# cgbur/llama2.zig

Measured on AMD Instinct MI355X. Metric: tokens/s (argmax, -t 0), higher is better.
Workload: dtype f32; 1 GPU; llama2-7b shape, fp32 llama2.c-v0 checkpoint (dim 4096, hidden 11008, L 32, H 32, kv 32, V 32000, S 2048), greedy from BOS, seeded synthetic weights; parallelism=1 GPU

## Files before the change

### llama2.zig_amd/csrc/kernel_common.h

```cpp
#pragma once
#include <cstdlib>

#include "l2z_comm.h"
#include "l2z_internal.h"
#include "tunables.h"

namespace l2z {
namespace {

constexpr int kWave = 64;
constexpr int kBlock = 256;
constexpr int kWaves = kBlock / kWave;
constexpr int kScratch = 32;

typedef float v4f __attribute__((ext_vector_type(4)));
typedef float v2f __attribute__((ext_vector_type(2)));

__device__ __forceinline__ v4f ldg_nt(const v4f *p) { return __builtin_nontemporal_load(p); }

__device__ __forceinline__ void block_copy_row(float *dst, const float *src, const int n, const int tid, const int n_threads)
{
    const int n4 = ((((uintptr_t)src | (uintptr_t)dst) & 15) == 0) ? n >> 2 : 0;
    for (int i = tid; i < n4; i += n_threads) ((v4f *)dst)[i] = ((const v4f *)src)[i];
    for (int i = 4 * n4 + tid; i < n; i += n_threads) dst[i] = src[i];
// ... 135 lines not shown
            ss = fmaf(v.x, v.x, ss);
            ss = fmaf(v.y, v.y, ss);
            ss = fmaf(v.z, v.z, ss);
            ss = fmaf(v.w, v.w, ss);
        }
    }
    if (PRO == PRO_RMS) {
        ss = wave_sum(ss);
        if ((tid & 63) == 0) scratch[tid >> 6] = ss;
        __syncthreads();
        float tot = scratch[0];
#pragma unroll
        for (int i = 1; i < kWaves; i++) tot += scratch[i];
        float s = tot / (float)n;
        s += 1e-5f;
        s = 1.0f / sqrtf(s);
        const v4f *g4 = (const v4f *)rms_w;
#pragma unroll
        for (int k = 0; k < XC; k++) {
            const int j = tid + kBlock * k;
            if (j < n4) {
                v4f v = xr[k];
                v.x = (v.x * s) * gr[k].x;
                v.y = (v.y * s) * gr[k].y;
                v.z = (v.z * s) * gr[k].z;
                v.w = (v.w * s) * gr[k].w;
                xs4[j] = v;
            }
        }
        for (int j = tid + kBlock * XC; j < n4; j += kBlock) {
            v4f v = xs4[j];
            const v4f g = g4[j];
            v.x = (v.x * s) * g.x;
            v.y = (v.y * s) * g.y;
            v.z = (v.z * s) * g.z;
            v.w = (v.w * s) * g.w;
            xs4[j] = v;
        }
    }
    __syncthreads();
}

template <int PRO, int XC>
__device__ __forceinline__ void xstage_finish(const float *__restrict__ x,
                                              const float *__restrict__ rms_w, int n, int n4_pad,
                                              v4f (&xr)[XC], v4f (&gr)[XC], float *xs,
                                              float *scratch)
{
    const v4f *x4 = (const v4f *)x;
    xstage_tail<PRO, XC>(rms_w, n, n4_pad, xr, gr, xs, scratch, [&](int j) { return x4[j]; });
}

struct LLPoll {
    const unsigned long long *slot;
    unsigned e;
    unsigned count;
    int *ctl;
    int *h_err;
    long long timeout_ticks;
};

__device__ __forceinline__ LLPoll ll_poll_init(const LLIn &in)
{
    LLPoll p;
    const int e = in.ctl[kCtlEpoch] + in.gi;
    p.e = (unsigned)e;
    p.slot = in.slots + (size_t)(e & 1) * in.slot_floats;
    p.count = in.count;
    p.ctl = in.ctl;
    p.h_err = in.h_err;
    p.timeout_ticks = in.timeout_ticks;
    return p;
}

__device__ __forceinline__ v4f ll_wait4(const LLPoll &p, int j, v4u a, v4u b)
{
    if (!(ll_ready2(a, p.e) && ll_ready2(b, p.e))) {
        bool give_up = __hip_atomic_load(p.ctl + kCtlErr, __ATOMIC_RELAXED, __HIP_MEMORY_SCOPE_AGENT) != 0;
        const long long t0 = wall_clock64();
        while (!give_up) {
            __builtin_amdgcn_s_sleep(16);
            a = ll_load2(p.slot, (size_t)4 * j);
            b = ll_load2(p.slot, (size_t)4 * j + 2);
            if (ll_ready2(a, p.e) && ll_ready2(b, p.e)) break;
            if (wall_clock64() - t0 > p.timeout_ticks) {
                give_up = true;
                __hip_atomic_store(p.ctl + kCtlErr, 1, __ATOMIC_RELAXED, __HIP_MEMORY_SCOPE_AGENT);
                *p.h_err = 1 + (int)((unsigned)(4 * j) / (p.count ? p.count : 1u));
            }
        }
    }
    v4f v;
    v.x = __uint_as_float(a.x);
    v.y = __uint_as_float(a.z);
    v.z = __uint_as_float(b.x);
    v.w = __uint_as_float(b.z);
    return v;
}

template <int PRO, int XC>
__device__ __forceinline__ void xload_issue_ll(const LLPoll &p, const float *__restrict__ rms_w,
                                               int n4, v4u (&xl)[2 * XC], v4f (&gr)[XC])
{
    const v4f *g4 = (const v4f *)rms_w;
#pragma unroll
    for (int k = 0; k < XC; k++) {
        const int j = threadIdx.x + kBlock * k;
        const int jc = j < n4 ? j : 0;
        xl[2 * k] = ll_load2(p.slot, (size_t)4 * jc);
        xl[2 * k + 1] = ll_load2(p.slot, (size_t)4 * jc + 2);
    }
    if (PRO == PRO_RMS) {
#pragma unroll
        for (int k = 0; k < XC; k++) {
            const int j = threadIdx.x + kBlock * k;
            gr[k] = (j < n4) ? g4[j] : v4f{0.f, 0.f, 0.f, 0.f};
        }
    }
}

template <int PRO, int XC>
__device__ __forceinline__ void xstage_finish_ll(const LLPoll &p, const float *__restrict__ rms_w,
                                                 int n, int n4_pad, v4u (&xl)[2 * XC],
                                                 v4f (&gr)[XC], float *xs, float *scratch)
{
    const int n4 = n >> 2;
    v4f xr[XC];
#pragma unroll
    for (int k = 0; k < XC; k++) {
        const int j = threadIdx.x + kBlock * k;
        const v4f v = ll_wait4(p, j < n4 ? j : 0, xl[2 * k], xl[2 * k + 1]);
        xr[k] = (j < n4) ? v : v4f{0.f, 0.f, 0.f, 0.f};
    }
    xstage_tail<PRO, XC>(rms_w, n, n4_pad, xr, gr, xs, scratch, [&](int j) {
        return ll_wait4(p, j, ll_load2(p.slot, (size_t)4 * j), ll_load2(p.slot, (size_t)4 * j + 2));
    });
}

template <int PRO, int XC, bool LL>
struct XStage {
    v4f xr[LL ? 1 : XC], gr[XC];
    v4u xl[LL ? 2 * XC : 2];
    LLPoll poll;

    __device__ __forceinline__ void issue(const float *x, const LLIn &xin, const float *rms_w, int n4)
    {
        if constexpr (LL) {
            poll = ll_poll_init(xin);
            xload_issue_ll<PRO, XC>(poll, rms_w, n4, xl, gr);
        } else {
            xload_issue<PRO, XC>(x, rms_w, n4, xr, gr);
        }
    }
    __device__ __forceinline__ void finish(const float *x, const float *rms_w, int n, int n4_pad, float *xs, float *scratch)
    {
        if constexpr (LL)
            xstage_finish_ll<PRO, XC>(poll, rms_w, n, n4_pad, xl, gr, xs, scratch);
        else
            xstage_finish<PRO, XC>(x, rms_w, n, n4_pad, xr, gr, xs, scratch);
    }
};

__device__ __forceinline__ void block_softmax(float *att, int T, float *scratch)
{
    const int tid = threadIdx.x, nt = blockDim.x;
    float m = -INFINITY;
    for (int t = tid; t < T; t += nt) m = fmaxf(m, att[t]);
    m = block_max(m, scratch);
    float s = 0.0f;
    for (int t = tid; t < T; t += nt) {
        const float e = expf(att[t] - m);
        att[t] = e;
        s += e;
    }
    s = block_sum(s, scratch);
    for (int t = tid; t < T; t += nt) att[t] = att[t] / s;
    __syncthreads();
}

struct AttnGeom {
    int E;
    int TPR;
    int G;
};

__host__ __device__ inline AttnGeom attn_geom(int head_size, bool vec, int block = kBlock)
{
    AttnGeom g;
    g.E = vec ? head_size >> 2 : head_size;
    int t = 1;
    while (t < g.E && t < 64) t <<= 1;
    g.TPR = t;
    g.G = block / t;
    return g;
}

__device__ __forceinline__ void wave_softmax(const float *att, float *prob, int T)
{
    const int lane = threadIdx.x & 63, wave = threadIdx.x >> 6, nw = blockDim.x >> 6;
    float m = -INFINITY;
    for (int t = lane; t < T; t += kWave) m = fmaxf(m, att[t]);
    m = wave_max(m);
    float s = 0.0f;
    for (int t = lane; t < T; t += kWave) s += expf(att[t] - m);
    s = wave_sum(s);
    for (int t = wave * kWave + lane; t < T; t += nw * kWave) prob[t] = expf(att[t] - m) / s;
    __syncthreads();
}

inline bool aligned16(const void *p) { return (reinterpret_cast<uintptr_t>(p) & 15u) == 0; }

template <typename K>
hipError_t ensure_lds(K kernel, size_t bytes)
{
    if (bytes > 64 * 1024) {
        hipError_t e = hipFuncSetAttribute(reinterpret_cast<const void *>(kernel),
                                           hipFuncAttributeMaxDynamicSharedMemorySize, (int)bytes);
        if (e != hipSuccess) return e;
    }
    return hipSuccess;
}

template <typename K, typename... Args>
hipError_t launch_lds(K kernel, dim3 grid, dim3 block, size_t lds, hipStream_t st, Args... args)
{
    hipError_t e = ensure_lds(kernel, lds);
    if (e != hipSuccess) return e;
    hipLaunchKernelGGL(kernel, grid, block, lds, st, args...);
    return hipGetLastError();
}

}
}
```

### llama2.zig_amd/csrc/l2z_internal.h

```cpp
#pragma once

#include <hip/hip_runtime.h>

#include <cstdarg>
#include <cstdint>
#include <cstdio>
#include <string>
#include <vector>

#include "../../include/llama2_hip.h"
#include "../../include/llama2_hip_test.h"

namespace l2z {

struct P2pArgs;

struct LLIn {
    const unsigned long long *slots;
    unsigned slot_floats;
    unsigned count;
    int gi;
    int *ctl;
    int *h_err;
    long long timeout_ticks;
};

void set_error(const char *fmt, ...);

#define L2Z_HIP(expr)                                                                    \
    do {                                                                                 \
        hipError_t _e = (expr);                                                          \
        if (_e != hipSuccess) {                                                          \
            ::l2z::set_error("%s failed: %s (%s:%d)", #expr, hipGetErrorString(_e),      \
                             __FILE__, __LINE__);                                        \
            return _e == hipErrorOutOfMemory ? L2Z_ERR_OOM                               \
                   : (_e == hipErrorNoDevice || _e == hipErrorInvalidDevice)             \
                       ? L2Z_ERR_NO_DEVICE                                               \
                       : L2Z_ERR_HIP;                                                    \
        }                                                                                \
    } while (0)

#define L2Z_CHECK(cond, code, ...)          \
    do {                                    \
        if (!(cond)) {                      \
            ::l2z::set_error(__VA_ARGS__);  \
            return (code);                  \
        }                                   \
    } while (0)

#define L2Z_TRY(expr)              \
    do {                           \
        int _s = (expr);           \
        if (_s != L2Z_OK) return _s; \
    } while (0)

template <class Sig> class FnRef;
template <class R, class... Args> class FnRef<R(Args...)> {
  public:
    template <class F>
    FnRef(const F &f) : f_(&f), call_([](const void *p, Args... args) -> R { return (*(const F *)p)(args...); }) {}
    R operator()(Args... args) const { return call_(f_, args...); }

  private:
    const void *f_;
    R (*call_)(const void *, Args...);
};


enum Prologue { PRO_NONE = 0, PRO_RMS = 1 };
enum Epilogue { EPI_STORE = 0, EPI_ROPE = 1, EPI_RESID = 2, EPI_SWIGLU = 3, EPI_ARGMAX = 4 };

constexpr int kMaxSeg = 3;

struct ArgmaxArgs {
    const float *logits;
    int vocab;
    const float *part_val;
    const int *part_idx;
    int n_part;
    int *token_ptr;
    int *pos_ptr;
    const int *prompt;
    const int *n_prompt_ptr;
    int *out_tokens;
    int *argmax_out;
    const float *tok_emb;
    float *x;
    int dim;
    int advance;
    int *epoch_ctl;
    int epoch_add;
    const P2pArgs *xchg;
    int xchg_gi;
};

struct MatvecArgs {
    const float *w0, *w1, *w2;
    float *out0, *out1, *out2;
    int rows0, rows1, rows2;
    int pos_stride1, pos_stride2;
    size_t kv_head_stride;
    int n;
    const float *x;
    const float *rms_w;
    const float *resid;
    const int *pos_ptr;
    const float2 *rope;
    int head_size;
    int rope_segs;
    float *part_val;
    int *part_idx;
    int row_offset;
    const P2pArgs *push;
    const int *push_ctl;
    int push_gi;
    LLIn xin;
    const uint32_t *pk, *pk1, *pk2;
    int pk_e, pk_e1, pk_e2;
    int tl_slot;
};

struct AttnArgs {
    const float *q;
    const float *kcache;
    const float *vcache;
    float *xb;
    const int *pos_ptr;
    int head_size;
    int kv_row;
    size_t kv_head;
    int kv_mul;
    int seq_len;
    const P2pArgs *push;
    const int *push_ctl;
    int push_gi;
    int tl_seq;
};


struct FusedQkvAttnArgs {
    const float *wq, *wk, *wv;
    const float *rms_w, *x;
    float *q_out;
    float *kcache, *vcache;
    float *xb;
    const int *pos_ptr;
    const float2 *rope;
    int n;
    int head_size, seq_len, kv_dim;
    int kv_row;
    size_t kv_head;
};
bool fused_qkv_attn_supported(int dim, int n_heads, int n_kv_heads, int seq_len, int n_cus);
hipError_t launch_fused_qkv_attn(const FusedQkvAttnArgs &a, int n_heads, hipStream_t st);

hipError_t launch_pk_stats(const float *m, size_t count, uint32_t *stats, hipStream_t st);
hipError_t launch_pk_pack(const float *m, int rows, int n, int e_base, uint32_t *pk, hipStream_t st);
hipError_t launch_pk_unpack(const uint32_t *pk, int rows, int n, int e_base, float *out, hipStream_t st);
hipError_t launch_matvec(const MatvecArgs &a, int pro, int epi, int max_blocks_per_cu, int n_cus,
                         hipStream_t st, int *out_grid = nullptr, bool *pushed = nullptr);
bool attention_push_supported(const AttnArgs &a);
int matvec_max_grid(int n_cus);
bool matvec_vector_width(int n);
hipError_t launch_stream_read(const float *p, size_t n_floats, float *out, int n_cus, hipStream_t st);
hipError_t launch_attention(const AttnArgs &a, int n_heads_local, hipStream_t st, int form = 0);
int attention_short_pos(int head_size, int seq_len);
int attention_split_chunks(int n_heads_local, int n_cus);
size_t attention_split_part_floats(int n_heads_local, int head_size, int nch);
bool attention_split_supported(const AttnArgs &a);
hipError_t launch_attention_split(const AttnArgs &a, int n_heads_local, int nch, float *part,
                                  int *arrivals, hipStream_t st, bool small = false);
int attention_split_wide_pos(int seq_len);
hipError_t launch_argmax(const ArgmaxArgs &a, hipStream_t st);
hipError_t launch_set_state(int token, int pos, int *token_ptr, int *pos_ptr, const float *tok_emb,
                            float *x, int dim, hipStream_t st);
hipError_t launch_rmsnorm(float *o, const float *x, const float *w, int n, hipStream_t st);
hipError_t launch_softmax(float *x, int n, hipStream_t st);
hipError_t launch_probs(float *probs, const float *logits, int n, float temperature, hipStream_t st);
hipError_t launch_dot(float *out, const float *x, const float *y, int n, hipStream_t st);
hipError_t launch_weighted_sum_rows(float *xout, int xout_len, const float *rows, int row_stride,
                                    const float *weights, int n_weights, hipStream_t st);
hipError_t launch_synth_fill(float *dst, uint64_t base_idx, uint64_t count, uint64_t seed,
                             float scale, float bias, hipStream_t st, uint64_t row_len = 0, uint64_t row_pitch = 0,
                             uint64_t idx_pitch = 0);
hipError_t launch_sum_parts(float *out, const float *const *parts, int n_parts, int n, hipStream_t st);
hipError_t launch_copy_rows(float *dst, size_t dpitch, const float *src, size_t rows, size_t cols, hipStream_t st);
size_t attention_lds_bytes(int head_size, int seq_len, bool vec);

struct SplitKWs {
    float *part;
    int *cnt;
    size_t part_floats;
    int cnt_ints;
    void *x3;
    size_t x3_bytes;
    void *x3b;
    size_t x3b_bytes;
};
struct DeferredSum {
    const float *part;
    int sk, feat, tm;
    bool valid;
};
enum PlanesReady { PLANES_SPLIT = 0, PLANES_READY = 1, PLANES_READY_B = 2 };
constexpr int kSplitKMaxTokens = 256;
constexpr int kPanelWsRows = 6 * kSplitKMaxTokens;
int prefill_split_k(long long n_whole, int P, int K, bool pair);
enum PrefillGemmEpi { PG_STORE = 0, PG_RESID = 1, PG_ROPE = 2, PG_ROPE_CACHE = 3, PG_CACHE = 4,
                      PG_SWIGLU = 5 };
bool x3_applies(long long n_whole, int K);
bool x3_stream_shape(long long n_whole, int P, int K);
int x3_stream_sk(long long n_whole, int P, int K);
enum GemmKind { GEMM_SINGLE = 0,
                GEMM_QKV,
                GEMM_W13,
                GEMM_KV };
struct GemmShape {
    int kind, epi;
    int P, N, K, ldx;
    int n_scale;
    long long n_launch_whole;
    int sk;
    int nq, nkv;
    int w13_one_matrix;
    size_t part_floats;
    int cnt_ints;
};
enum GemmFamily { GF_INVALID = -1, GF_NOT_SUPPORTED = -2, GF_NO_WORKSPACE = -3,
                  GF_STREAM = 1,
                  GF_SHORT,
                  GF_SPLIT_K,
                  GF_TWO_BLOCK,
                  GF_TILE };
enum TileForm { TILE_128x64 = 0, TILE_64x64, TILE_32x64, TILE_32x32, TILE_128x128 };
struct GemmPlan {
    int family;
    int epi;
    int K;
    int x3;
    int sk;
    int tile;
    int feat, tm, nbuf, one_round;
    int tms, paired;
};
GemmPlan prefill_gemm_plan(const GemmShape &s);
hipError_t launch_prefill_rmsnorm(float *o, int ldo, const float *x, const float *w, int n, int P,
                                  hipStream_t st,
                                  void *x3 = nullptr, int kp = 0,
                                  const DeferredSum *pending = nullptr,
                                  const int *rows = nullptr);
hipError_t launch_prefill_embed(float *x, const float *tok_emb, const int *tokens, int dim, int P,
                                hipStream_t st);
hipError_t launch_prefill_attention(const float *q, int ldq, const float *kcache, const float *vcache,
                                    float *out, int ldo, int pos0, int P, int n_heads, int head_size,
                                    int kv_row, size_t kv_head, int kv_mul, int seq_len, hipStream_t st,
                                    int n_heads_model = 0,
                                    int form = 0,
                                    void *x3 = nullptr, int kp = 0,
                                    bool *planes_written = nullptr);
constexpr int kRaggedMaxSeq = 16;
struct RaggedSeq {
    float *kc, *vc;
    int row0, rows;
    int pos0;
    int pad;
    const int32_t *pages;
};
__device__ __forceinline__ int kv_page_id(const int32_t *pages, int i)
{
    return ((const __attribute__((address_space(4))) int32_t *)pages)[i];
// ... 69 lines not shown
```

### llama2.zig_amd/csrc/matvec.hip

```cpp
#include <type_traits>

#include "argmax_rule.h"
#include "matvec_device.h"
#include "packed_w.h"

namespace l2z {
namespace {

__device__ __forceinline__ void dot2_scalar(const float *__restrict__ pa,
                                            const float *__restrict__ pb, const float *xs, int n,
                                            float &ra, float &rb)
{
    const int lane = threadIdx.x & 63;
    float sa = 0.0f, sb = 0.0f;
    for (int j = lane; j < n; j += kWave) {
        const float xv = xs[j];
        sa = fmaf(pa[j], xv, sa);
        sb = fmaf(pb[j], xv, sb);
    }
    ra = wave_sum(sa);
    rb = wave_sum(sb);
}

template <int LPR>
// ... 28 lines not shown
        acc_a = fma4(wa[k], xv, acc_a);
        acc_b = fma4(wb[k], xv, acc_b);
    }
}

struct MvStep {
    bool unit_done, more;
    int u_next, b_next;
};

__device__ __forceinline__ MvStep mv_step(int u, int b, int n_batches, int ustride, int n_units)
{
    MvStep s;
    s.unit_done = (b + 1 == n_batches);
    s.u_next = s.unit_done ? u + ustride : u;
    s.b_next = s.unit_done ? 0 : b + 1;
    s.more = s.u_next < n_units;
    return s;
}

template <int PRO, int EPI, int LPR, int XC, bool LL>
__global__ __launch_bounds__(kBlock) void matvec_kernel(const MatvecArgs a)
{
    using G = MvGeom<LPR>;
    constexpr int U = G::U, RW = G::RW;
    extern __shared__ __attribute__((aligned(16))) float lds[];
    const MvLocals m = mv_locals<EPI>(a);
    const int n4 = m.n >> 2;
    const int n_batches = (n4 + LPR * U - 1) / (LPR * U);
    const int n4_pad = n_batches * (LPR * U);
    float *xs = lds;
    float *scratch = lds + 4 * n4_pad;
    const v4f *xs4 = (const v4f *)xs;

    const int lane = threadIdx.x & 63, wave = threadIdx.x >> 6;
    const int grp = lane / LPR, cl = lane % LPR;
    const int n_units = (m.n_pairs + RW - 1) / RW;
    const int ustride = gridDim.x * kWaves;

    XStage<PRO, XC, LL> xst;
    xst.issue(a.x, a.xin, a.rms_w, n4);
    int u = blockIdx.x * kWaves + wave;
    const bool has_unit = u < n_units;
    const float *pa, *pb;
    pair_rows<EPI>(m, (has_unit ? u : 0) * RW + grp, pa, pb);
    v4f wa[U], wb[U];
    EpiIn ein = epi_prefetch<EPI>(m, (has_unit ? u : 0) * RW + grp, cl == 0 && has_unit);
    EpiIn ein_next = ein;
    mv_load<LPR>(pa, pb, cl, n4, wa, wb);
    xst.finish(a.x, a.rms_w, m.n, n4_pad, xs, scratch);
    if (EPI != EPI_ARGMAX && !has_unit) return;

    v4f acc_a = {0.f, 0.f, 0.f, 0.f}, acc_b = {0.f, 0.f, 0.f, 0.f};
    ArgmaxCand best;
    int b = 0;
    while (has_unit) {
        mv_consume<LPR>(xs4, cl + b * (LPR * U), wa, wb, acc_a, acc_b);
        const MvStep s = mv_step(u, b, n_batches, ustride, n_units);
        if (s.more) {
            if (s.unit_done) {
                pair_rows<EPI>(m, s.u_next * RW + grp, pa, pb);
                ein_next = epi_prefetch<EPI>(m, s.u_next * RW + grp, cl == 0);
            }
            mv_load<LPR>(pa, pb, cl + s.b_next * (LPR * U), n4, wa, wb);
        }
        if (s.unit_done) {
            const float sa = lanes_sum(hsum4(acc_a), LPR);
            const float sb = lanes_sum(hsum4(acc_b), LPR);
            pair_epilogue<EPI>(m, u * RW + grp, sa, sb, cl == 0, ein);
            ein = ein_next;
            if (EPI == EPI_ARGMAX) {
                const int ra_ = 2 * (u * RW + grp), rb_ = ra_ + 1;
                if (ra_ < m.total_rows) argmax_take(best, sa, ra_ + a.row_offset);
                if (rb_ < m.total_rows) argmax_take(best, sb, rb_ + a.row_offset);
            }
            acc_a = v4f{0.f, 0.f, 0.f, 0.f};
            acc_b = v4f{0.f, 0.f, 0.f, 0.f};
        }
        if (!s.more) break;
        u = s.u_next;
        b = s.b_next;
    }
    if (EPI == EPI_ARGMAX) {
        argmax_wave_fold(best);
        __syncthreads();
        if (lane == 0) {
            scratch[wave] = best.v;
            scratch[kWaves + wave] = __int_as_float(best.i);
        }
        __syncthreads();
        if (threadIdx.x == 0) {
            ArgmaxCand c = {scratch[0], __float_as_int(scratch[kWaves])};
            for (int w = 1; w < kWaves; w++) argmax_merge(c, scratch[w], __float_as_int(scratch[kWaves + w]));
            a.part_val[blockIdx.x] = c.v;
            a.part_idx[blockIdx.x] = c.i;
        }
    }
}

struct PkRaw {
    v4u q4[7];
    uint32_t q1[3];
};

__device__ __forceinline__ void pk_load_raw(const uint32_t *src, int lane, int s, PkRaw &r)
{
    const int q = pk::lane_dw(s) / 4, rem = pk::lane_dw(s) % 4;
#pragma unroll
    for (int i = 0; i < 7; i++)
        if (i < q) r.q4[i] = __builtin_nontemporal_load((const v4u *)(src + i * 256 + lane * 4));
#pragma unroll
    for (int i = 0; i < 3; i++)
        if (i < rem) r.q1[i] = __builtin_nontemporal_load(src + q * 256 + i * 64 + lane);
}

template <int S>
__device__ __forceinline__ void pk_decode_lane(const PkRaw &r, int e31, v4f (&wa)[4], v4f (&wb)[4])
{
    constexpr int N = pk::lane_dw(S), Q = N / 4;
    uint32_t d[N > 0 ? N : 1], t[8 * S > 0 ? 8 * S : 1];
#pragma unroll
    for (int i = 0; i < N; i++) {
        if (i < 4 * Q) {
            const v4u v = r.q4[i / 4];
            d[i] = (i % 4 == 0) ? v.x : (i % 4 == 1) ? v.y : (i % 4 == 2) ? v.z : v.w;
        } else {
            d[i] = r.q1[i - 4 * Q];
        }
    }
    pk::decode_lane_t<S>(d, t);
#pragma unroll
    for (int k = 0; k < 4; k++) {
        if (k < S) {
            wa[k] = v4f{__builtin_amdgcn_ldexpf(__uint_as_float(t[8 * k]), e31), __builtin_amdgcn_ldexpf(__uint_as_float(t[8 * k + 1]), e31),
                        __builtin_amdgcn_ldexpf(__uint_as_float(t[8 * k + 2]), e31), __builtin_amdgcn_ldexpf(__uint_as_float(t[8 * k + 3]), e31)};
            wb[k] = v4f{__builtin_amdgcn_ldexpf(__uint_as_float(t[8 * k + 4]), e31), __builtin_amdgcn_ldexpf(__uint_as_float(t[8 * k + 5]), e31),
                        __builtin_amdgcn_ldexpf(__uint_as_float(t[8 * k + 6]), e31), __builtin_amdgcn_ldexpf(__uint_as_float(t[8 * k + 7]), e31)};
        } else {
            wa[k] = v4f{0.f, 0.f, 0.f, 0.f};
            wb[k] = v4f{0.f, 0.f, 0.f, 0.f};
        }
    }
}

constexpr int kRowU = 4;

template <int EPI, int XC>
struct RowF32 {
    static constexpr int kSets = 1;
    v4f wa[kRowU], wb[kRowU];
    const float *pa, *pb;
    int n4;

    __device__ __forceinline__ void init(const MvLocals &, int n4_, int) { n4 = n4_; }
    __device__ __forceinline__ void point(const MvLocals &m, int u) { pair_rows<EPI>(m, u, pa, pb); }
    template <int P>
    __device__ __forceinline__ void issue(int b)
    {
        const int tid = threadIdx.x, cb = b * (kBlock * kRowU);
        const v4f *a4 = (const v4f *)pa + cb + tid, *b4 = (const v4f *)pb + cb + tid;
        const int wbase = cb + (tid & ~63);
#pragma unroll
        for (int k = 0; k < kRowU; k++) {
            const bool in_row = wbase + kBlock * k < n4;
            if (XC == 12 && !in_row) {
                wa[k] = v4f{0.f, 0.f, 0.f, 0.f};
                wb[k] = v4f{0.f, 0.f, 0.f, 0.f};
                continue;
            }
            const int off = in_row ? kBlock * k : -(cb + (tid & ~63));
            wa[k] = ldg_nt(a4 + off);
            wb[k] = ldg_nt(b4 + off);
        }
    }
    template <int P>
    __device__ __forceinline__ void deliver() {}
};

template <int EPI, int XC>
struct RowPacked {
    static constexpr int kSets = 2;
    v4f wa[kRowU], wb[kRowU];
    PkRaw raw[kSets];
    int s_in[kSets], e31[kSets];
    const uint32_t *pp;
    size_t pdw, last_off;
    int e_pt, s_last, wave_u, n_batches;

    __device__ __forceinline__ void init(const MvLocals &, int n4, int n_batches_)
    {
        n_batches = n_batches_;
        wave_u = __builtin_amdgcn_readfirstlane(threadIdx.x >> 6);
        pdw = pk::pair_dw(n4);
        last_off = pk::chunk_off(n4, n_batches - 1, wave_u);
        s_last = pk::steps(n4, n_batches - 1, wave_u);
    }
    __device__ __forceinline__ void point(const MvLocals &m, int u)
    {
        int e;
        pp = pair_packed<EPI>(m, u, pdw, e);
        e_pt = e - 31;
    }
    template <int P>
    __device__ __forceinline__ void issue(int b)
    {
        const bool last = b + 1 == n_batches;
        const uint32_t *src = pp + (last ? last_off : (size_t)b * (4 * 64 * pk::kMaxLaneDw) + (size_t)wave_u * (64 * pk::kMaxLaneDw));
        s_in[P] = (XC == 4 || !last) ? 4 : s_last;
        e31[P] = e_pt;
        pk_load_raw(src, threadIdx.x & 63, XC == 4 ? 4 : s_in[P], raw[P]);
    }
    template <int P>
    __device__ __forceinline__ void deliver()
    {
        if constexpr (XC == 4) {
            pk_decode_lane<4>(raw[P], e31[P], wa, wb);
        } else {
            switch (s_in[P]) {
                case 4: pk_decode_lane<4>(raw[P], e31[P], wa, wb); break;
                case 3: pk_decode_lane<3>(raw[P], e31[P], wa, wb); break;
                case 2: pk_decode_lane<2>(raw[P], e31[P], wa, wb); break;
                case 1: pk_decode_lane<1>(raw[P], e31[P], wa, wb); break;
                default: pk_decode_lane<0>(raw[P], e31[P], wa, wb); break;
            }
        }
    }
};

#ifdef L2Z_TIMELINE
constexpr int kMtlSlots = 256, kMtlBlocks = 512;
__device__ long long g_mtl[kMtlSlots * kMtlBlocks * 8];
unsigned long long g_mtl_launches = 0;
#define L2Z_MTL(i) tl[i] = wall_clock64()
#else
#define L2Z_MTL(i) do { } while (0)
#endif

template <int PRO, int EPI, int XC, bool LL, bool PK = false>
__global__ __launch_bounds__(kBlock) void matvec_row_kernel(const MatvecArgs a)
{
    constexpr int U = kRowU;
    using Src = typename std::conditional<PK, RowPacked<EPI, XC>, RowF32<EPI, XC>>::type;
    constexpr int NS = Src::kSets;
    extern __shared__ __attribute__((aligned(16))) float lds[];
#ifdef L2Z_TIMELINE
    long long tl[8] = {0, 0, 0, 0, 0, 0, 0, 0};
#endif
    L2Z_MTL(0);
    MvLocals m_ = mv_locals<EPI>(a);
    if constexpr (PK) m_.push = nullptr;
    const MvLocals m = m_;
    const int n4 = m.n >> 2;
    const int n_batches = (n4 + kBlock * U - 1) / (kBlock * U);
    const int n4_pad = n_batches * (kBlock * U);
    float *xs = lds;
    float *scratch = lds + 4 * n4_pad;
    float *part = scratch + kScratch;
    const v4f *xs4 = (const v4f *)xs;
    const int tid = threadIdx.x, lane = tid & 63, wave = tid >> 6;
    const int n_units = m.n_pairs;
    const int ustride = gridDim.x;

    XStage<PRO, XC, LL> xst;
    xst.issue(a.x, a.xin, a.rms_w, n4);
    int u = blockIdx.x;
    Src src;
    src.init(m, n4, n_batches);
    src.point(m, u);
    EpiIn ein = epi_prefetch<EPI>(m, u, tid == 0);
    EpiIn ein_next = ein;
    src.template issue<0>(0);
    L2Z_MTL(1);
    xst.finish(a.x, a.rms_w, m.n, n4_pad, xs, scratch);
    L2Z_MTL(2);

    int iu = u, ib = 0;
    bool imore = true;
    auto advance = [&]() __attribute__((always_inline)) {
        const MvStep s = mv_step(iu, ib, n_batches, ustride, n_units);
        imore = s.more;
        if (s.more) {
            if (s.unit_done) src.point(m, s.u_next);
            iu = s.u_next;
            ib = s.b_next;
        }
    };
    advance();

    v4f acc_a = {0.f, 0.f, 0.f, 0.f}, acc_b = {0.f, 0.f, 0.f, 0.f};
    ArgmaxCand best;
    int b = 0, parity = 0;
    auto step = [&](auto set, auto ahead) __attribute__((always_inline)) -> bool {
        constexpr int P = decltype(set)::value;
        const MvStep s = mv_step(u, b, n_batches, ustride, n_units);
        auto prefetch_next = [&]() __attribute__((always_inline)) {
            if (s.more && s.unit_done) ein_next = epi_prefetch<EPI>(m, s.u_next, tid == 0);
        };
        if constexpr (NS > 1) {
            prefetch_next();
            if constexpr (decltype(ahead)::value) {
                if constexpr (EPI == EPI_SWIGLU) asm volatile("s_waitcnt vmcnt(0)" ::: "memory");
                src.template issue<(P + 1) % NS>(ib);
                advance();
            }
        }
        src.template deliver<P>();
#pragma unroll
        for (int k = 0; k < U; k++) {
            const v4f xv = xs4[b * (kBlock * U) + tid + kBlock * k];
            acc_a = fma4(src.wa[k], xv, acc_a);
            acc_b = fma4(src.wb[k], xv, acc_b);
        }
        if constexpr (NS == 1) {
            prefetch_next();
            if (imore) {
                src.template issue<0>(ib);
                advance();
            }
        }
#ifdef L2Z_TIMELINE
        tl[6]++;
#endif
        if (s.unit_done) {
            const float sa = wave_sum(hsum4(acc_a));
            const float sb = wave_sum(hsum4(acc_b));
            float *pp_ = part + parity * (2 * kWaves);
            if (lane == 0) {
                pp_[wave] = sa;
                pp_[kWaves + wave] = sb;
            }
            __syncthreads();
            if (tid == 0) {
                const float ta = ((pp_[0] + pp_[1]) + pp_[2]) + pp_[3];
                const float tb = ((pp_[kWaves] + pp_[kWaves + 1]) + pp_[kWaves + 2]) + pp_[kWaves + 3];
                pair_epilogue<EPI>(m, u, ta, tb, true, ein);
                if (EPI == EPI_ARGMAX) {
                    const int ra_ = 2 * u, rb_ = ra_ + 1;
                    argmax_take(best, ta, ra_ + a.row_offset);
                    if (rb_ < m.total_rows) argmax_take(best, tb, rb_ + a.row_offset);
                }
            }
            ein = ein_next;
            parity ^= 1;
            acc_a = v4f{0.f, 0.f, 0.f, 0.f};
            acc_b = v4f{0.f, 0.f, 0.f, 0.f};
#ifdef L2Z_TIMELINE
            if (tl[7]++ == 0) L2Z_MTL(3);
            L2Z_MTL(4);
#endif
        }
        u = s.u_next;
        b = s.b_next;
        return !s.more;
    };
    using Set0 = std::integral_constant<int, 0>;
    using Set1 = std::integral_constant<int, 1>;
    static_assert(NS == 1 || NS == 2, "register sets of a source");
    if constexpr (NS == 1) {
        while (!step(Set0{}, std::false_type{})) {}
    } else {
        while (true) {
            if (!imore) { step(Set0{}, std::false_type{}); break; }
            step(Set0{}, std::true_type{});
            if (!imore) { step(Set1{}, std::false_type{}); break; }
            step(Set1{}, std::true_type{});
        }
    }
    if (EPI == EPI_ARGMAX && tid == 0) {
        a.part_val[blockIdx.x] = best.v;
        a.part_idx[blockIdx.x] = best.i;
    }
#ifdef L2Z_TIMELINE
    L2Z_MTL(5);
    if (tid == 0 && (unsigned)a.tl_slot < (unsigned)kMtlSlots && blockIdx.x < kMtlBlocks) {
        long long *o = g_mtl + ((size_t)a.tl_slot * kMtlBlocks + blockIdx.x) * 8;
        for (int i = 0; i < 8; i++) o[i] = tl[i];
    }
#endif
}

template <int PRO, int EPI>
__global__ __launch_bounds__(kBlock) void matvec_scalar_kernel(const MatvecArgs a)
{
    extern __shared__ __attribute__((aligned(16))) float lds[];
    const MvLocals m = mv_locals<EPI>(a);
    float *xs = lds;
    float *scratch = lds + ((m.n + 3) & ~3);
    stage_x_scalar<PRO>(a.x, a.rms_w, m.n, xs, scratch);
    const int lane = threadIdx.x & 63, wave = threadIdx.x >> 6;
    for (int u = blockIdx.x * kWaves + wave; u < m.n_pairs; u += gridDim.x * kWaves) {
        const float *pa, *pb;
        pair_rows<EPI>(m, u, pa, pb);
        float sa, sb;
        dot2_scalar(pa, pb, xs, m.n, sa, sb);
        pair_epilogue<EPI>(m, u, sa, sb, lane == 0, epi_prefetch<EPI>(m, u, lane == 0));
    }
}

int lpr_for(int n4)
{
    int l = 8;
    while (l < 64 && l * 6 < n4) l <<= 1;
    return l;
}

struct MvLaunch {
    const void *fn;
    int lpr, u;
};

template <int PRO, int EPI, int LPR, int XC, bool LL>
MvLaunch mv_entry()
{
    return {reinterpret_cast<const void *>(&matvec_kernel<PRO, EPI, LPR, XC, LL>), LPR, MvGeom<LPR>::U};
}

template <int PRO, int EPI, bool LL>
MvLaunch mv_pick(int lpr, bool big_x)
{
    if (lpr == 8) return mv_entry<PRO, EPI, 8, 4, LL>();
    if (lpr == 16) return mv_entry<PRO, EPI, 16, 4, LL>();
    if (lpr == 32) return mv_entry<PRO, EPI, 32, 4, LL>();
    return big_x ? mv_entry<PRO, EPI, 64, 12, LL>() : mv_entry<PRO, EPI, 64, 4, LL>();
}

template <int PRO, int EPI, bool LL, bool PK = false>
const void *mv_row_fn(bool big_x)
{
    return big_x ? reinterpret_cast<const void *>(&matvec_row_kernel<PRO, EPI, 12, LL, PK>)
                 : reinterpret_cast<const void *>(&matvec_row_kernel<PRO, EPI, 4, LL, PK>);
}

#define L2Z_MV_COMBOS(X)                     \
    X(PRO_NONE, EPI_STORE,  0, 1, 0)         \
    X(PRO_NONE, EPI_RESID,  1, 1, 1)         \
    X(PRO_RMS,  EPI_STORE,  1, 1, 0)         \
    X(PRO_RMS,  EPI_ROPE,   1, 1, 1)         \
    X(PRO_RMS,  EPI_SWIGLU, 1, 1, 1)         \
    X(PRO_RMS,  EPI_ARGMAX, 1, 0, 1)
#define L2Z_IF_1(...) __VA_ARGS__
#define L2Z_IF_0(...)

const void *mv_row_pick_packed(int pro, int epi, bool big_x)
{
#define X(P, E, LL, SC, PK) L2Z_IF_##PK(if (pro == P && epi == E) return mv_row_fn<P, E, false, true>(big_x);)
    L2Z_MV_COMBOS(X)
#undef X
    return nullptr;
}

const void *mv_row_pick(int pro, int epi, bool big_x, bool ll)
{
#define X(P, E, LL, SC, PK)                                           \
    if (pro == P && epi == E && !ll) return mv_row_fn<P, E, false>(big_x); \
    L2Z_IF_##LL(if (pro == P && epi == E && ll) return mv_row_fn<P, E, true>(big_x);)
    L2Z_MV_COMBOS(X)
#undef X
    return nullptr;
}

MvLaunch mv_pick_pe(int pro, int epi, int lpr, bool big_x, bool vec, bool ll)
{
#define X(P, E, LL, SC, PK)                                                                \
    if (pro == P && epi == E && vec && !ll) return mv_pick<P, E, false>(lpr, big_x);       \
    L2Z_IF_##LL(if (pro == P && epi == E && vec && ll) return mv_pick<P, E, true>(lpr, big_x);) \
    L2Z_IF_##SC(if (pro == P && epi == E && !vec && !ll)                                   \
                    return MvLaunch{reinterpret_cast<const void *>(&matvec_scalar_kernel<P, E>), 0, 0};)
    L2Z_MV_COMBOS(X)
#undef X
    return {nullptr, 0, 0};
}
#undef L2Z_MV_COMBOS
#undef L2Z_IF_1
#undef L2Z_IF_0

__global__ __launch_bounds__(256) void stream_read_kernel(const v4f *__restrict__ p, size_t n4, float *out)
{
    constexpr int U = 8;
    size_t i = (size_t)blockIdx.x * 256 * U + threadIdx.x;
    const size_t stride = (size_t)gridDim.x * 256 * U;
    v4f acc = {0.f, 0.f, 0.f, 0.f};
    for (; i + 256 * (U - 1) < n4; i += stride) {
        v4f r[U];
#pragma unroll
        for (int k = 0; k < U; k++) r[k] = ldg_nt(p + i + 256 * k);
#pragma unroll
        for (int k = 0; k < U; k++) acc += r[k];
    }
    const float s = (acc.x + acc.y) + (acc.z + acc.w);
    if (s == 123.456f) out[blockIdx.x] = s;
}

}

size_t matvec_lds_bytes(int n) { return (size_t)(4 * ((n >> 2) + 1024) + kScratch + 4 * kWaves + 4) * sizeof(float); }

int matvec_max_grid(int n_cus) { return n_cus * 8; }

bool matvec_vector_width(int n) { return n > 0 && (n % 4) == 0; }

hipError_t launch_stream_read(const float *p, size_t n_floats, float *out, int n_cus, hipStream_t st)
{
    hipLaunchKernelGGL(stream_read_kernel, dim3(n_cus * 8), dim3(256), 0, st, (const v4f *)p, n_floats / 4, out);
    return hipGetLastError();
}

hipError_t launch_matvec(const MatvecArgs &a_in, int pro, int epi, int max_blocks_per_cu, int n_cus,
                         hipStream_t st, int *out_grid, bool *pushed)
{
    MatvecArgs a = a_in;
    if (max_blocks_per_cu > 8) max_blocks_per_cu = 8;
    bool vec = (a.n % 4) == 0 && aligned16(a.x) && aligned16(a.w0);
    if (a.rows1 > 0) vec = vec && aligned16(a.w1);
    if (a.rows2 > 0) vec = vec && aligned16(a.w2);
    if (pro == PRO_RMS) vec = vec && aligned16(a.rms_w);
    if (epi == EPI_SWIGLU && a.rows1 != a.rows0) return hipErrorInvalidValue;
    const int total_rows = a.rows0 + a.rows1 + a.rows2;
    const int n_pairs = (epi == EPI_SWIGLU) ? a.rows0 : (total_rows + 1) / 2;
    if (n_pairs <= 0 || a.n <= 0) return hipErrorInvalidValue;
    const int n4 = a.n >> 2;
    const int lpr = lpr_for(n4);
    if (epi == EPI_ARGMAX && (!vec || a.rows1 != 0 || a.rows2 != 0)) return hipErrorNotSupported;
    const Tunables &tn = tunables();
    const bool use_row = vec && n4 >= 1024 && (n4 % 64) == 0;
    const bool ll = a.xin.slots != nullptr;
    if (ll && !vec) return hipErrorNotSupported;
    if (a.pk != nullptr && (!use_row || ll || !pk::width_ok(a.n))) return hipErrorInvalidValue;
    if (a.pk != nullptr) a.push = nullptr;
    if (a.pk != nullptr && epi != EPI_SWIGLU &&
        ((a.rows1 > 0 && a.pk1 == nullptr) || (a.rows2 > 0 && a.pk2 == nullptr) || a.rows0 % 2 || a.rows1 % 2 || a.rows2 % 2))
        return hipErrorInvalidValue;
    MvLaunch k = {nullptr, 0, 0};
    size_t lds;
    int n_units;
    const auto padded = [n4](int batch) { return ((n4 + batch - 1) / batch) * batch; };
    if (use_row) {
        k.fn = a.pk != nullptr ? mv_row_pick_packed(pro, epi, a.n > 4096) : mv_row_pick(pro, epi, a.n > 4096, ll);
        lds = (size_t)(4 * padded(kBlock * kRowU) + kScratch + 4 * kWaves) * sizeof(float);
        n_units = n_pairs;
    } else if (vec) {
        k = mv_pick_pe(pro, epi, lpr, a.n > 4096, true, ll);
        if (k.fn == nullptr) return hipErrorInvalidValue;
        lds = (size_t)(4 * padded(k.lpr * k.u) + kScratch) * sizeof(float);
        const int rw = kWave / k.lpr;
        n_units = (n_pairs + rw - 1) / rw;
    } else {
        k = mv_pick_pe(pro, epi, lpr, a.n > 4096, false, ll);
        lds = (size_t)(((a.n + 3) & ~3) + kScratch) * sizeof(float);
        n_units = n_pairs;
    }
    if (k.fn == nullptr) return hipErrorInvalidValue;
    if (lds > 64 * 1024) {
        hipError_t e = hipFuncSetAttribute(k.fn, hipFuncAttributeMaxDynamicSharedMemorySize, (int)lds);
        if (e != hipSuccess) return e;
    }
    int occ = 0;
    if (hipOccupancyMaxActiveBlocksPerMultiprocessor(&occ, k.fn, kBlock, lds) != hipSuccess || occ < 1)
        occ = 1;
    if (occ > max_blocks_per_cu) occ = max_blocks_per_cu;
    if (use_row && occ > tn.row_blocks) occ = tn.row_blocks;
    int resident = occ * n_cus;
    if (tn.grid_cap > 0 && resident > tn.grid_cap) resident = tn.grid_cap;
    int grid;
    if (use_row) {
        grid = n_units;
        if (grid > resident) {
            const int per_block = (n_units + resident - 1) / resident;
            grid = (n_units + per_block - 1) / per_block;
        }
    } else {
        const int blocks_needed = (n_units + kWaves - 1) / kWaves;
        grid = blocks_needed;
        if (grid > resident) {
            const int per_wave = (n_units + resident * kWaves - 1) / (resident * kWaves);
            grid = (n_units + per_wave * kWaves - 1) / (per_wave * kWaves);
        }
    }
    if (out_grid) *out_grid = grid;
    if (!vec || epi == EPI_ROPE || a.rows2 != 0 || (epi != EPI_SWIGLU && a.rows1 != 0)) a.push = nullptr;
    if (pushed) *pushed = a.push != nullptr;
#ifdef L2Z_TIMELINE
    a.tl_slot = use_row ? (int)(g_mtl_launches++ % kMtlSlots) : -1;
#endif
    void *args[] = {&a};
    return hipLaunchKernel(k.fn, dim3(grid), dim3(kBlock), args, lds, st);
}

}

#ifdef L2Z_TIMELINE
extern "C" int l2z_matvec_timeline_dump(long long *out, unsigned long long *n_launches)
{
    if (hipDeviceSynchronize() != hipSuccess) return 1;
    if (hipMemcpyFromSymbol(out, HIP_SYMBOL(l2z::g_mtl), sizeof(long long) * l2z::kMtlSlots * l2z::kMtlBlocks * 8) != hipSuccess) return 1;
    *n_launches = l2z::g_mtl_launches;
    return 0;
}
#endif
```

### llama2.zig_amd/csrc/matvec_device.h

```cpp
#pragma once
#include "kernel_common.h"

namespace l2z {
namespace {

struct MvLocals {
    const float *w0, *w1, *w2;
    float *out0, *out1, *out2;
    const float *resid;
    const float2 *rope;
    int rows0, r01, total_rows, n_pairs, n, head_size, rope_segs, pos;
    size_t ps1, ps2;
    size_t kv_head_stride;
    const P2pArgs *push;
    int push_e;
    size_t push_base;
    const uint32_t *pk, *pk1, *pk2;
    int pk_e, pk_e1, pk_e2;
};

template <int EPI>
__device__ __forceinline__ MvLocals mv_locals(const MatvecArgs &a)
{
    MvLocals m;
    m.w0 = a.w0; m.w1 = a.w1; m.w2 = a.w2;
    m.out0 = a.out0; m.out1 = a.out1; m.out2 = a.out2;
    m.resid = a.resid; m.rope = a.rope;
    m.rows0 = a.rows0; m.r01 = a.rows0 + a.rows1; m.total_rows = a.rows0 + a.rows1 + a.rows2;
    m.n_pairs = (EPI == EPI_SWIGLU) ? a.rows0 : (m.total_rows + 1) >> 1;
    m.n = a.n; m.head_size = a.head_size; m.rope_segs = a.rope_segs;
    m.pos = (EPI == EPI_ROPE) ? *a.pos_ptr : 0;
    m.ps1 = (size_t)m.pos * (size_t)a.pos_stride1;
    m.ps2 = (size_t)m.pos * (size_t)a.pos_stride2;
    m.kv_head_stride = (EPI == EPI_ROPE) ? a.kv_head_stride : 0;
    m.push = a.push;
    m.push_e = m.push ? a.push_ctl[kCtlEpoch] + a.push_gi : 0;
    m.push_base = m.push ? (size_t)m.push->rank * m.push->count : 0;
    m.pk = a.pk; m.pk1 = a.pk1; m.pk2 = a.pk2;
    m.pk_e = a.pk_e; m.pk_e1 = a.pk_e1; m.pk_e2 = a.pk_e2;
    return m;
}

struct SegRow {
    bool past0, past1;
    int row;
    __device__ __forceinline__ int seg() const { return past1 ? 2 : (past0 ? 1 : 0); }
    template <typename T>
    __device__ __forceinline__ T pick(T v0, T v1, T v2) const
    {
        const T v = past0 ? v1 : v0;
        return past1 ? v2 : v;
    }
};

__device__ __forceinline__ SegRow seg_row(const MvLocals &m, int g)
{
    SegRow r;
    r.past0 = g >= m.rows0;
    r.past1 = g >= m.r01;
    r.row = g - (r.past1 ? m.r01 : (r.past0 ? m.rows0 : 0));
    return r;
}

template <int EPI>
__device__ __forceinline__ void pair_rows(const MvLocals &m, int p, const float *&pa, const float *&pb)
{
    if (p >= m.n_pairs) p = m.n_pairs - 1;
    if (EPI == EPI_SWIGLU) {
        pa = m.w0 + (size_t)(2 * p) * (size_t)m.n;
        pb = pa + m.n;
    } else {
        const int ga = 2 * p;
        const int gb = (ga + 1 < m.total_rows) ? ga + 1 : ga;
        const SegRow ra = seg_row(m, ga), rb = seg_row(m, gb);
        pa = ra.pick(m.w0, m.w1, m.w2) + (size_t)ra.row * (size_t)m.n;
        pb = rb.pick(m.w0, m.w1, m.w2) + (size_t)rb.row * (size_t)m.n;
    }
}

template <int EPI>
__device__ __forceinline__ const uint32_t *pair_packed(const MvLocals &m, int p, size_t pair_dw, int &e_base)
{
    if (p >= m.n_pairs) p = m.n_pairs - 1;
    if (EPI == EPI_ROPE) {
        const SegRow r = seg_row(m, 2 * p);
        e_base = r.pick(m.pk_e, m.pk_e1, m.pk_e2);
        return r.pick(m.pk, m.pk1, m.pk2) + (size_t)(r.row >> 1) * pair_dw;
    }
    e_base = m.pk_e;
    return m.pk + (size_t)p * pair_dw;
}

struct EpiIn {
    float ra, rb;
    float2 cs;
};

template <int EPI>
__device__ __forceinline__ EpiIn epi_prefetch(const MvLocals &m, int p, bool writer)
{
    EpiIn e;
    e.ra = 0.0f; e.rb = 0.0f; e.cs = make_float2(1.0f, 0.0f);
    if (!writer || p >= m.n_pairs) return e;
    if (EPI == EPI_RESID) {
        const int ga = 2 * p, gb = ga + 1;
        e.ra = m.resid[ga];
        if (gb < m.total_rows) e.rb = m.resid[gb];
    } else if (EPI == EPI_ROPE) {
        const SegRow ra = seg_row(m, 2 * p);
        if (ra.seg() < m.rope_segs) {
            const int hs = m.head_size;
            e.cs = m.rope[(size_t)m.pos * (size_t)(hs >> 1) + (size_t)((ra.row % hs) >> 1)];
        }
    }
    return e;
}

template <int EPI>
__device__ __forceinline__ void pair_epilogue(const MvLocals &m, int p, float sa, float sb, bool writer, const EpiIn &in)
{
    const bool valid_a = p < m.n_pairs;
    if (EPI == EPI_SWIGLU) {
        float v = sa;
        v = v * (1.0f / (1.0f + expf(-v)));
        v = v * sb;
        if (writer && valid_a) {
            m.out0[p] = v;
            if (m.push) p2p_ll_push(m.push, m.push_e, m.push_base + (size_t)p, v);
        }
        return;
    }
    const int ga = 2 * p, gb = ga + 1;
    const bool valid_b = valid_a && gb < m.total_rows;
    const SegRow ra = seg_row(m, ga), rb = seg_row(m, gb);
    const int row_a = ra.row, row_b = rb.row;
    float *oa = ra.pick(m.out0, m.out1 + m.ps1, m.out2 + m.ps2);
    float *ob = rb.pick(m.out0, m.out1 + m.ps1, m.out2 + m.ps2);
    if (EPI == EPI_ROPE) {
        float o0 = sa, o1 = sb;
        if (ra.seg() < m.rope_segs) {
            const float2 cs = in.cs;
            o0 = sa * cs.x - sb * cs.y;
            o1 = sa * cs.y + sb * cs.x;
        }
        if (writer && valid_a) {
            size_t ia = (size_t)row_a, ib = (size_t)row_b;
            if (m.kv_head_stride) {
                const int hs = m.head_size;
                if (ra.past0) ia = (size_t)(row_a / hs) * m.kv_head_stride + (size_t)(row_a % hs);
                if (rb.past0) ib = (size_t)(row_b / hs) * m.kv_head_stride + (size_t)(row_b % hs);
            }
            oa[ia] = o0;
            if (valid_b) ob[ib] = o1;
        }
    } else if (EPI == EPI_RESID) {
        if (writer && valid_a) {
            const float va = in.ra + sa, vb = in.rb + sb;
            oa[row_a] = va;
            if (valid_b) ob[row_b] = vb;
            if (m.push) {
                p2p_ll_push(m.push, m.push_e, m.push_base + (size_t)row_a, va);
                if (valid_b) p2p_ll_push(m.push, m.push_e, m.push_base + (size_t)row_b, vb);
            }
        }
    } else {
        if (writer && valid_a) {
            oa[row_a] = sa;
            if (valid_b) ob[row_b] = sb;
            if (m.push) {
                p2p_ll_push(m.push, m.push_e, m.push_base + (size_t)row_a, sa);
                if (valid_b) p2p_ll_push(m.push, m.push_e, m.push_base + (size_t)row_b, sb);
            }
        }
    }
}

}
}
```

Measured before the change: 244.0 tokens/s.

## Issue x, rms and first packed weight loads before computing matvec locals

Reorders the packed-weight matvec prologue so the first weight chunk, the whole x/rms vector and the residual values are loaded before the remaining kernel arguments are decoded. The pos pointer read for RoPE is moved after the x stage finishes. MatvecArgs is reordered so the fields needed first sit together, and the packed pair stride is computed on the host. The aim is to shorten the latency-bound startup of each matvec block, at the cost of more live registers in the prologue and extra code-path variants.

Result: no change. 243.6 tokens/s, median of 2 (-0.2%).

```diff
diff --git a/llama2.zig_amd/csrc/kernel_common.h b/llama2.zig_amd/csrc/kernel_common.h
--- a/llama2.zig_amd/csrc/kernel_common.h
+++ b/llama2.zig_amd/csrc/kernel_common.h
@@ -311,6 +311,16 @@
             xload_issue<PRO, XC>(x, rms_w, n4, xr, gr);
         }
     }
+    __device__ __forceinline__ void issue_whole(const float *x, const float *rms_w)
+    {
+        static_assert(!LL, "plain x only");
+#pragma unroll
+        for (int k = 0; k < XC; k++) xr[k] = ((const v4f *)x)[threadIdx.x + kBlock * k];
+        if constexpr (PRO == PRO_RMS) {
+#pragma unroll
+            for (int k = 0; k < XC; k++) gr[k] = ((const v4f *)rms_w)[threadIdx.x + kBlock * k];
+        }
+    }
     __device__ __forceinline__ void finish(const float *x, const float *rms_w, int n, int n4_pad, float *xs, float *scratch)
     {
         if constexpr (LL)
diff --git a/llama2.zig_amd/csrc/l2z_internal.h b/llama2.zig_amd/csrc/l2z_internal.h
--- a/llama2.zig_amd/csrc/l2z_internal.h
+++ b/llama2.zig_amd/csrc/l2z_internal.h
@@ -95,15 +95,17 @@
 };
 
 struct MatvecArgs {
+    const uint32_t *pk, *pk1, *pk2;
+    int rows0, rows1, rows2;
+    int n;
+    unsigned pk_pair_dw;
     const float *w0, *w1, *w2;
-    float *out0, *out1, *out2;
-    int rows0, rows1, rows2;
-    int pos_stride1, pos_stride2;
-    size_t kv_head_stride;
-    int n;
     const float *x;
     const float *rms_w;
     const float *resid;
+    float *out0, *out1, *out2;
+    int pos_stride1, pos_stride2;
+    size_t kv_head_stride;
     const int *pos_ptr;
     const float2 *rope;
     int head_size;
@@ -115,7 +117,6 @@
     const int *push_ctl;
     int push_gi;
     LLIn xin;
-    const uint32_t *pk, *pk1, *pk2;
     int pk_e, pk_e1, pk_e2;
     int tl_slot;
 };
diff --git a/llama2.zig_amd/csrc/matvec.hip b/llama2.zig_amd/csrc/matvec.hip
--- a/llama2.zig_amd/csrc/matvec.hip
+++ b/llama2.zig_amd/csrc/matvec.hip
@@ -204,7 +204,11 @@
     const float *pa, *pb;
     int n4;
 
-    __device__ __forceinline__ void init(const MvLocals &, int n4_, int) { n4 = n4_; }
+    __device__ __forceinline__ void init(const MvLocals &m, int n4_, int, int u)
+    {
+        n4 = n4_;
+        point(m, u);
+    }
     __device__ __forceinline__ void point(const MvLocals &m, int u) { pair_rows<EPI>(m, u, pa, pb); }
     template <int P>
     __device__ __forceinline__ void issue(int b)
@@ -239,13 +243,22 @@
     size_t pdw, last_off;
     int e_pt, s_last, wave_u, n_batches;
 
-    __device__ __forceinline__ void init(const MvLocals &, int n4, int n_batches_)
+    __device__ __forceinline__ void first(const MvLocals &h, int u)
+    {
+        wave_u = __builtin_amdgcn_readfirstlane(threadIdx.x >> 6);
+        pdw = XC == 4 ? (size_t)(4 * 64 * pk::kMaxLaneDw) : h.pk_pair_dw;
+        int e;
+        pp = pair_packed<EPI>(h, u, pdw, e);
+        s_in[0] = 4;
+        pk_load_raw(pp + (size_t)wave_u * (64 * pk::kMaxLaneDw), threadIdx.x & 63, 4, raw[0]);
+    }
+    __device__ __forceinline__ void init(const MvLocals &m, int n4, int n_batches_, int u)
     {
         n_batches = n_batches_;
-        wave_u = __builtin_amdgcn_readfirstlane(threadIdx.x >> 6);
-        pdw = pk::pair_dw(n4);
         last_off = pk::chunk_off(n4, n_batches - 1, wave_u);
         s_last = pk::steps(n4, n_batches - 1, wave_u);
+        point(m, u);
+        e31[0] = e_pt;
     }
     __device__ __forceinline__ void point(const MvLocals &m, int u)
     {
@@ -299,9 +312,26 @@
     long long tl[8] = {0, 0, 0, 0, 0, 0, 0, 0};
 #endif
     L2Z_MTL(0);
-    MvLocals m_ = mv_locals<EPI>(a);
-    if constexpr (PK) m_.push = nullptr;
-    const MvLocals m = m_;
+    constexpr bool kXFirst = PK && XC == 4 && EPI != EPI_SWIGLU;
+    const int tid = threadIdx.x, lane = tid & 63, wave = tid >> 6;
+    int u = blockIdx.x;
+    Src src;
+    XStage<PRO, XC, LL> xst;
+    EpiIn ein = {0.0f, 0.0f, make_float2(1.0f, 0.0f)};
+    if constexpr (PK) {
+        if constexpr (kXFirst) {
+            xst.issue_whole(a.x, a.rms_w);
+            if constexpr (EPI == EPI_RESID) {
+                ein.ra = a.resid[2 * u];
+                ein.rb = a.resid[2 * u + 1];
+            }
+        }
+        src.first(mv_head<EPI>(a), u);
+        __builtin_amdgcn_sched_barrier(0);
+        L2Z_MTL(1);
+    }
+    MvLocals m = mv_locals<EPI, !kXFirst>(a);
+    if constexpr (PK) m.push = nullptr;
     const int n4 = m.n >> 2;
     const int n_batches = (n4 + kBlock * U - 1) / (kBlock * U);
     const int n4_pad = n_batches * (kBlock * U);
@@ -309,22 +339,26 @@
     float *scratch = lds + 4 * n4_pad;
     float *part = scratch + kScratch;
     const v4f *xs4 = (const v4f *)xs;
-    const int tid = threadIdx.x, lane = tid & 63, wave = tid >> 6;
     const int n_units = m.n_pairs;
     const int ustride = gridDim.x;
 
-    XStage<PRO, XC, LL> xst;
-    xst.issue(a.x, a.xin, a.rms_w, n4);
-    int u = blockIdx.x;
-    Src src;
-    src.init(m, n4, n_batches);
-    src.point(m, u);
-    EpiIn ein = epi_prefetch<EPI>(m, u, tid == 0);
-    EpiIn ein_next = ein;
-    src.template issue<0>(0);
-    L2Z_MTL(1);
+    if constexpr (!kXFirst) xst.issue(a.x, a.xin, a.rms_w, n4);
+    if constexpr (PK) {
+        src.init(m, n4, n_batches, u);
+        if constexpr (!kXFirst) ein = epi_prefetch<EPI>(m, u, tid == 0);
+    } else {
+        src.init(m, n4, n_batches, u);
+        ein = epi_prefetch<EPI>(m, u, tid == 0);
+        src.template issue<0>(0);
+        L2Z_MTL(1);
+    }
     xst.finish(a.x, a.rms_w, m.n, n4_pad, xs, scratch);
     L2Z_MTL(2);
+    if constexpr (kXFirst && EPI == EPI_ROPE) {
+        mv_set_pos<EPI>(m, a);
+        ein = epi_prefetch<EPI>(m, u, tid == 0);
+    }
+    EpiIn ein_next = ein;
 
     int iu = u, ib = 0;
     bool imore = true;
@@ -579,6 +613,7 @@
     if (ll && !vec) return hipErrorNotSupported;
     if (a.pk != nullptr && (!use_row || ll || !pk::width_ok(a.n))) return hipErrorInvalidValue;
     if (a.pk != nullptr) a.push = nullptr;
+    a.pk_pair_dw = a.pk != nullptr ? (unsigned)pk::pair_dw(n4) : 0u;
     if (a.pk != nullptr && epi != EPI_SWIGLU &&
         ((a.rows1 > 0 && a.pk1 == nullptr) || (a.rows2 > 0 && a.pk2 == nullptr) || a.rows0 % 2 || a.rows1 % 2 || a.rows2 % 2))
         return hipErrorInvalidValue;
diff --git a/llama2.zig_amd/csrc/matvec_device.h b/llama2.zig_amd/csrc/matvec_device.h
--- a/llama2.zig_amd/csrc/matvec_device.h
+++ b/llama2.zig_amd/csrc/matvec_device.h
@@ -17,28 +17,46 @@
     size_t push_base;
     const uint32_t *pk, *pk1, *pk2;
     int pk_e, pk_e1, pk_e2;
+    size_t pk_pair_dw;
 };
 
 template <int EPI>
+__device__ __forceinline__ MvLocals mv_head(const MatvecArgs &a)
+{
+    MvLocals m = {};
+    m.w0 = a.w0; m.w1 = a.w1; m.w2 = a.w2;
+    m.rows0 = a.rows0; m.r01 = a.rows0 + a.rows1; m.total_rows = a.rows0 + a.rows1 + a.rows2;
+    m.n_pairs = (EPI == EPI_SWIGLU) ? a.rows0 : (m.total_rows + 1) >> 1;
+    m.n = a.n;
+    m.pk = a.pk; m.pk1 = a.pk1; m.pk2 = a.pk2;
+    m.pk_pair_dw = a.pk_pair_dw;
+    return m;
+}
+
+template <int EPI, bool POS = true>
 __device__ __forceinline__ MvLocals mv_locals(const MatvecArgs &a)
 {
-    MvLocals m;
-    m.w0 = a.w0; m.w1 = a.w1; m.w2 = a.w2;
+    MvLocals m = mv_head<EPI>(a);
     m.out0 = a.out0; m.out1 = a.out1; m.out2 = a.out2;
     m.resid = a.resid; m.rope = a.rope;
-    m.rows0 = a.rows0; m.r01 = a.rows0 + a.rows1; m.total_rows = a.rows0 + a.rows1 + a.rows2;
-    m.n_pairs = (EPI == EPI_SWIGLU) ? a.rows0 : (m.total_rows + 1) >> 1;
-    m.n = a.n; m.head_size = a.head_size; m.rope_segs = a.rope_segs;
-    m.pos = (EPI == EPI_ROPE) ? *a.pos_ptr : 0;
+    m.head_size = a.head_size; m.rope_segs = a.rope_segs;
+    m.pos = (EPI == EPI_ROPE && POS) ? *a.pos_ptr : 0;
     m.ps1 = (size_t)m.pos * (size_t)a.pos_stride1;
     m.ps2 = (size_t)m.pos * (size_t)a.pos_stride2;
     m.kv_head_stride = (EPI == EPI_ROPE) ? a.kv_head_stride : 0;
     m.push = a.push;
     m.push_e = m.push ? a.push_ctl[kCtlEpoch] + a.push_gi : 0;
     m.push_base = m.push ? (size_t)m.push->rank * m.push->count : 0;
-    m.pk = a.pk; m.pk1 = a.pk1; m.pk2 = a.pk2;
     m.pk_e = a.pk_e; m.pk_e1 = a.pk_e1; m.pk_e2 = a.pk_e2;
     return m;
+}
+
+template <int EPI>
+__device__ __forceinline__ void mv_set_pos(MvLocals &m, const MatvecArgs &a)
+{
+    m.pos = (EPI == EPI_ROPE) ? *a.pos_ptr : 0;
+    m.ps1 = (size_t)m.pos * (size_t)a.pos_stride1;
+    m.ps2 = (size_t)m.pos * (size_t)a.pos_stride2;
 }
 
 struct SegRow {
```
